# montyhall/bot7

Measured on AMD Instinct MI355X. Metric: EI candidates scored/sec at N=2048,d=32, higher is better.
Workload: dtype f64

## Files before the change

### bot7_amd/csrc/b7_internal.h

```cpp
#pragma once
#include <hip/hip_runtime.h>
#include <stddef.h>
#include <stdint.h>

#include <map>
#include <string>
#include <vector>

#include "bot7hip.h"

constexpr int B7_NPAD = 128;
constexpr int B7_PANEL = 64;
constexpr int B7_PERSIST_NMAX = 4096;
constexpr int B7_MROWS = 256;
constexpr int B7_MAX_D = 96;

constexpr int B7_TAB_VAL = 0;
constexpr int B7_TAB_IDX = 1;
constexpr int B7_TAB_STATUS = 2;
constexpr int B7_TAB_ROWS = 3;
constexpr int B7_TAB_ROW0 = 4;
constexpr int B7_TAB_W = B7_TAB_ROW0 + B7_MAX_D;
constexpr int B7_MAX_WORLD = 64;

static inline int b7_dpad_class(int d) {
  return d <= 4 ? 4 : d <= 8 ? 8 : d <= 16 ? 16 : d <= 32 ? 32 : d <= 48 ? 48 : d <= 64 ? 64 : 96;
}

constexpr size_t B7_INFO_HEAD_BYTES = 16 + sizeof(double) * 257 + 8;
constexpr size_t B7_PERSIST_FLAG_WORDS_MAX = 16 + 2 * 64 * 64 + 2 * 64;
constexpr size_t B7_INFO_BYTES = B7_INFO_HEAD_BYTES + 4 * B7_PERSIST_FLAG_WORDS_MAX;

struct DevBuf {
  void *p = nullptr;
  size_t cap = 0;
};

struct PinBuf {
  void *host = nullptr, *dev = nullptr;
  size_t bytes = 0;
};

struct FitBlock { int info[4]; double terms[257]; };
struct BestPair { double v; int64_t i; };
constexpr int SOBOL_DIMS = 40;
constexpr int SOBOL_BITS = 30;
struct SobolTable {
  uint32_t v[SOBOL_DIMS][SOBOL_BITS];
};

constexpr size_t B7_PINNED_BYTES = 16384;
struct PinnedBlock {
  FitBlock fit;
  alignas(256) BestPair best;
  alignas(4096) double fmin[256];
  alignas(4096) double vec[B7_MAX_D + 3];
};
static_assert(offsetof(PinnedBlock, fit) == 0 && offsetof(PinnedBlock, best) == 2304 && offsetof(PinnedBlock, fmin) == 4096 &&
                  offsetof(PinnedBlock, vec) == 8192 && sizeof(PinnedBlock) <= B7_PINNED_BYTES,
              "pinned block: kernels and copies address these slots");

constexpr size_t B7_SCRATCH_BYTES = 64 * 1024;
struct ScratchBlock {
  double lenscale[256];
  double fmin[256];
  SobolTable sobol;
  double minmax[2 * B7_MAX_D];
  alignas(4096) double colvec[2 * B7_MAX_D];
};
static_assert(offsetof(ScratchBlock, lenscale) == 0 && offsetof(ScratchBlock, fmin) == 2048 && offsetof(ScratchBlock, sobol) == 4096 &&
                  offsetof(ScratchBlock, minmax) == 4096 + sizeof(SobolTable) && offsetof(ScratchBlock, colvec) == 12288 &&
                  sizeof(ScratchBlock) <= B7_SCRATCH_BYTES,
              "scratch block: the layout every earlier build used");

constexpr int B7_ACC_NONE = 0, B7_ACC_LINEAR = 1, B7_ACC_LOG = 2;

struct PhaseStat {
  double ms = 0.0;
  int64_t launches = 0;
};

struct ScoreParams {
  int kind = 0, S = 0, upper = 0, nlev = 0;
  const double *mu = nullptr, *var = nullptr;
  union {
    const double *fmin = nullptr;
    const double *ystar;
  };
  long long stride = 0;
  double fmin0 = 0.0, tradeoff = 0.0, sign = 0.0;
};

struct b7_ctx {
  int device = 0;
  hipStream_t stream = nullptr;
  hipEvent_t ev_fit = nullptr;
  std::string err;
  int cus = 0;

  DevBuf grid[2];
  int grid_cur = 0;
  int64_t M = 0;
  int d = 0;

  bool fitted = false;
  bool have_data = false;
  int model_kind = 0;
  int N = 0, Npad = 0, dfit = 0, dpad = 0, ycols = 0;
  int yld = 1;
  double amp = 0, noise = 0, mean = 0;
  b7_gp_opts opts;
  int kernel = B7_KERNEL_ARDSE;
  DevBuf xobs;
  DevBuf w;
  DevBuf zsc;
  DevBuf zss;
  DevBuf K;
  DevBuf L;
  DevBuf Linv;
  DevBuf W;
  DevBuf dinv;
  DevBuf alpha;
  DevBuf resid;
  DevBuf atmp;
  DevBuf info;
  DevBuf ybuf;

  bool predicted = false;
  int64_t Mpred = 0;
  DevBuf mu;
  DevBuf var;
  DevBuf acc;
  bool acc_valid = false;
  int spin_us = 500;
  bool npad_small = true;
  bool potrf_small = true;
  bool blr_small = true;
  double fmin_scalar = 0.0;
  bool acc_fresh = false;
  int acc_kind = 0;
  DevBuf ks;
  size_t ks_bytes = (size_t)4 << 30;
  int diag_variant = 1;
  int inverse_inline = 1;
  PinnedBlock *pinned = nullptr, *pinned_dev = nullptr;
  std::vector<double> net_host;
  PinBuf pin_blr;
  PinBuf pin_eval;
  PinBuf pin_nll;
  bool fmin_staged = false;
  bool potrf_attrs_set = false;
  bool linv_done = false;
  int potrf_sched = 3;
  int syrk_small = 1;
  int potrf_defer = 1;
  int potrf_group = 2;
  struct JobList { DevBuf buf; int n = 0; };
  std::map<int, JobList> pjobs_cache;
  DevBuf pstamps;
  int pjobs_nb = 0, pjobs_n = 0;
  DevBuf bhyp, bw, bzsc, bzss, bK, bL, bdinv, bflags, binfo, bresid, bterms, bLinv, balpha, bmu, bvar;
  bool persist_attr_set = false, persist_stamps = false;
  int persist_helpers = 0;
  int persist_aborts = 0;
  int nll_small = 1;
  bool kpost_small = true;
  bool fit_small = true;
  int persist_fault = -1;
  int potrf_sched_saved = 0;
  DevBuf part;
  DevBuf ystar, mes_ticket;
  DevBuf mes_user;
  int mes_levels = 8;
  int mes_S = 0, mes_K = 0, mes_nb = 0;
  int64_t mes_M = 0;
  int mes_slot = 0;
  bool mes_valid = false;
  DevBuf ticket;
  DevBuf scratch;
  DevBuf tmpgrid;
  DevBuf tmpmu, tmpvar;
  DevBuf fant;
  DevBuf bel;
  DevBuf belvec;
  PinBuf pin_bel;
  DevBuf feat;
  size_t feat_zeroed_bytes = 0;
  int feat_z = -1;
  int64_t Mfeat = 0;
  int zdim = 0;
  uint64_t feat_version = 0, grid_version = 0;
  DevBuf netbuf;

  void *comm = nullptr;
  int comm_rank = 0, comm_world = 1;
  DevBuf slots;
  uint64_t *tab_host = nullptr;
  uint64_t *tab_host_dev = nullptr;
  struct b7_group *group = nullptr;
  bool group_busy = false;
  bool win_valid = false;
  int64_t win_idx1 = 0;
  int win_rank = -1, win_d = 0;
  double win_row[B7_MAX_D];
  int64_t shard_rows[B7_MAX_WORLD];
  int shard_world = 0;

  hipEvent_t tev[B7_MAX_TIMERS][2];
  bool tev_init = false;
  bool profile = false;
  std::map<std::string, PhaseStat> phases;
  struct PendingPhase { const char *name; hipEvent_t e0, e1; };
  std::vector<PendingPhase> pending;
  std::vector<hipEvent_t> free_events;
  hipEvent_t phase_e0 = nullptr;
};

int b7_fail(b7_ctx *c, int code, const char *fmt, ...);
#define B7_HIP(c, expr)                                                                          \
  do {                                                                                           \
    hipError_t e__ = (expr);                                                                     \
    if (e__ != hipSuccess)                                                                       \
      return b7_fail((c), e__ == hipErrorOutOfMemory ? B7_ERR_NOMEM : B7_ERR_HIP, "%s:%d: %s", \
                     __FILE_NAME__, __LINE__, hipGetErrorString(e__));                           \
  } while (0)
#define B7_TRY(expr)          \
  do {                        \
    int rc__ = (expr);        \
    if (rc__ != B7_OK) return rc__; \
  } while (0)

int b7_ensure(b7_ctx *c, DevBuf &b, size_t bytes);
void b7_release(DevBuf &b);
int b7_pin_ensure(b7_ctx *c, PinBuf &b, size_t bytes, bool mapped);
static inline ScratchBlock *b7_scratch(const b7_ctx *c) { return static_cast<ScratchBlock *>(c->scratch.p); }

struct PhaseScope {
  b7_ctx *c;
  const char *name;
  PhaseScope(b7_ctx *c, const char *name);
  ~PhaseScope();
};

static inline int64_t round_up(int64_t x, int64_t m) { return (x + m - 1) / m * m; }
int npad_of(const b7_ctx *c, int64_t n);

int launch_sobol(b7_ctx *c, double *out, int64_t size, int dims, int64_t skip, const double *mins,
                 const double *maxes);
int launch_random_grid(b7_ctx *c, double *out, int64_t size, int dims, uint64_t seed, int64_t row_offset,
                       const double *mins, const double *maxes);
int launch_remove_row(b7_ctx *c, const double *src, double *dst, int64_t M, int d, int64_t idx0);
int launch_remove_rows(b7_ctx *c, const double *src, double *dst, int64_t M, int d, const int64_t *cuts_dev, int ncut);
int launch_colrange(b7_ctx *c, const double *grid, int64_t M, int d, double *out_dev);
int launch_col_affine(b7_ctx *c, double *grid, int64_t M, int d, const double *v_dev, bool mul);
int launch_gather_rows(b7_ctx *c, const double *src, double *out, const int64_t *idx0_dev, int64_t n, int d);

struct KBatchDesc {
  int64_t s_w = 0, s_zsc = 0, s_zsh = 0, s_out = 0;
  const double *amp = nullptr;
  int64_t s_alpha = 0, s_mu = 0;
  const double *mean = nullptr;
};
struct ObsSet {
  const double *zsc;
  const double *zsh;
  int npad;
  const double *w = nullptr;
  KBatchDesc batch;
};
int launch_prep_obs_aux(b7_ctx *c, const double *xobs, const double *ls_dev, int N, int npad, double *zsc,
                        double *zsh);
int launch_k_generic(b7_ctx *c, const double *xq, int64_t rows, int64_t Mtotal, const ObsSet &o, double *out);
int launch_prep_obs(b7_ctx *c, const double *xobs, const double *lenscale_sq_dev, int N, int d);
int launch_kxx(b7_ctx *c, double diag_add);
int launch_ksx_batch(b7_ctx *c, int S, const double *xq, int64_t rows, int64_t Mtotal, const double *w, const double *zsc,
                     const double *zss, const double *amp_dev, const double *mean_dev, const double *alpha, double *ks,
                     int64_t s_out, double *mu, int64_t s_mu);
int launch_kxx_batch(b7_ctx *c, int B, const double *ls_dev, const double *amp_dev, const double *noise_dev, double *w,
                     double *zsc, double *zss, double *K);
int launch_ksx(b7_ctx *c, const double *xq, int64_t row0, int64_t rows, int64_t Mtotal, int d, double *ks,
               double *mu, int ycols);

struct FactorNote {
  bool alpha_done = false;
  int *report_written = nullptr;
};
int launch_potrf(b7_ctx *c, double extra, bool with_inverse, int *report_hint = nullptr, FactorNote *note = nullptr);
int launch_trtri(b7_ctx *c);
int launch_potrf_persist(b7_ctx *c, double extra, bool with_inverse);
int launch_nll_batch(b7_ctx *c, int B, const double *K, double *L, double *dinv, unsigned *flags, int *info,
                     const double *resid, double *terms);
int launch_nll_one(b7_ctx *c, const double *K, double *L, double *dinv, unsigned *flags, int *info, const double *resid,
                   double *terms, double extra);
size_t persist_flag_words_host(int nb);
int launch_potrf_small(b7_ctx *c, int B, const double *K, double *L, double *Linv, double *dinv, const double *resid, double *alpha,
                       double extra, int *info, int *report_dev, int64_t sK, int64_t sL, int64_t sdinv, int64_t svec, int sinfo);
int launch_blr_head_small(b7_ctx *c, const double *Z, int N, int z, int ldz, const double *yv, double alpha_prec, double beta,
                          int *report_dev);
int launch_blr_heads_small(b7_ctx *c, int S, const double *Z, int N, int z, int ldz, const double *yraw_dev, const double *hyp3_dev,
                           double *L, double *Linv, double *m, double *b, int *info, int *report_dev, double *terms);
int launch_post_heads(b7_ctx *c, int S, const double *Linv, const double *feat, int64_t rows, int64_t Mtotal, double *var, int64_t svar,
                      const double *zero_dev, const double *invbeta_dev);
int launch_gemv_rows_batch(b7_ctx *c, int S, const double *A, int lda, const double *x, int64_t sx, int n, const double *base_dev,
                           int64_t rows, double *y, int64_t sy);
int launch_nll_small(b7_ctx *c, int B, const double *hyp_dev, const double *hyp_host, double *terms_dev, int *info_dev,
                     unsigned *done_dev);
bool kpost_small_applies(const b7_ctx *c);
int launch_kpost_small(b7_ctx *c, int S, const double *xq, int64_t M, const double *w, const double *zsc, const double *zss,
                       const double *Linv, const double *alpha, const double *hyp_dev, double amp, double noise, double mean,
                       double *mu, double *var, int64_t sout);
bool gp_small_applies(const b7_ctx *c);
static inline bool fit_small_applies(const b7_ctx *c) {
  return c->fit_small && c->potrf_sched == 3 && c->inverse_inline && gp_small_applies(c);
}
int launch_nll_small8(b7_ctx *c, int B, const double *hyp_dev, const double *hyp_host, double *terms_dev, int *info_dev,
                      unsigned *done_dev);
int launch_fit_small(b7_ctx *c, int B, const double *hyp_dev, const double *hyp_host, double *hyp_out, double *w, double *zsc,
                     double *zss, double *L, double *Linv, double *dinv, double *alpha, double *resid, int *info_dev,
                     int *report_dev);
int launch_alpha(b7_ctx *c, int *report_dev = nullptr, int report_words = 0, const FactorNote &note = FactorNote());
int launch_alpha_batch(b7_ctx *c, int B, const double *Linv, const double *resid, double *alpha, const int *report_src = nullptr,
                       int *report_dev = nullptr, int report_words = 0);
int launch_fit_batch(b7_ctx *c, int B, const double *K, double *L, double *Linv, double *dinv, unsigned *flags, int *info);
int launch_nll_terms(b7_ctx *c, double *out_dev);
int launch_fro_norm_sq(b7_ctx *c, const double *A, int n, int ld, double *out_dev);
int launch_set_identity(b7_ctx *c);

int launch_post(b7_ctx *c, const double *ks, int64_t row0, int64_t rows, int64_t Mtotal, double *var);
int launch_post_batch(b7_ctx *c, int S, const double *Linv, const double *ks, int64_t sks, int64_t rows, int64_t Mtotal,
                      double *var, int64_t svar, const double *amp_dev, const double *noise_dev);

int launch_mean_multi(b7_ctx *c, const double *ks, int64_t row0, int64_t rows, int64_t Mtotal, double *mu);
int launch_gemm_nt(b7_ctx *c, const double *A, int lda, const double *B, int ldb, double *C, int ldc, int m, int n,
                   int k);
int launch_fantasy_cov(b7_ctx *c, const double *kpp, const double *g, double *S, int P, double diag_add);
int launch_fantasy_factor(b7_ctx *c, double *S, double *dinv_tmp, int *info_dev);
int launch_fantasy_sample(b7_ctx *c, const double *Lp, const double *mu, int P, int n, uint64_t seed, double *out);
int launch_add_diag(b7_ctx *c, double *S, int ld, int n, double v);

int launch_append_finalize(b7_ctx *c, const double *krow, const double *lvec, const double *uvec, const double *evec,
                           int *status_dev);
int launch_append_vectors(b7_ctx *c, const double *krow, double *lvec, double *uvec, double *part, double *evec);
int launch_mlp_forward(b7_ctx *c, const double *X, int64_t M, int d, const double *net_dev, const int *dims,
                       int n_layers, int activation, double *out, int ld_out);
int launch_mlp_forward_mean(b7_ctx *c, const double *X, int64_t M, int d, const double *net_dev, const int *dims,
                            int n_layers, int activation, double *out, int ld_out, const double *mvec, double mean0,
                            double *mu, bool *mean_done);
int launch_gemv_rows(b7_ctx *c, const double *A, int lda, const double *x, int n, double base, int64_t row0,
                     int64_t rows, int64_t Mtotal, double *y);
int launch_transpose_pad(b7_ctx *c, const double *Z, int n, int ldz, int z, double *Zt, int zpad, int nk);
int launch_blr_assemble(b7_ctx *c, const double *G, double *K, int z, int zpad, double alpha_prec, double beta);

int launch_score(b7_ctx *c, ScoreParams p, const double *mu, const double *var, int64_t M, int ycols, double *out, bool accumulate);
int launch_score_batch(b7_ctx *c, const ScoreParams &p, double *acc, int64_t M);
int launch_finish(b7_ctx *c, double *acc, int64_t M, double divisor, double *best_val, int64_t *best_idx1, bool logacc = false);
int launch_fill(b7_ctx *c, double *p, int64_t n, double v);
int launch_finish_slot(b7_ctx *c, double *acc, int64_t M, double divisor, uint64_t *tab_dev, int rank, int world,
                       int64_t offset, const double *grid, int d, bool all_slots, uint64_t *host_rec = nullptr,
                       unsigned *host_done = nullptr, bool logacc = false);

struct ExclRows {
  int n = 0;
  long long row[B7_BATCH_MAX];
};
int launch_score_finish_slot(b7_ctx *c, const ScoreParams &p, double *acc, int64_t M, double divisor, uint64_t *tab_dev,
                             int rank, int world, int64_t offset, const double *grid, int d, bool all_slots, uint64_t *host_rec = nullptr,
                             unsigned *host_done = nullptr, const ExclRows *excl = nullptr);
void acc_declare_zeros(b7_ctx *c, int score_kind);
int acc_write_zeros(b7_ctx *c);
void acc_forget(b7_ctx *c);
int acc_materialize(b7_ctx *c);
int launch_keep_record(b7_ctx *c, uint64_t *tab_dev, int rank, int world);
int launch_row_slot(b7_ctx *c, uint64_t *tab_dev, int rank, int world, int64_t idx1_global, int64_t local0, const double *grid,
                    int d);

int exch_table_ensure(b7_ctx *c, int world);
int exch_local(b7_ctx *c, double divisor, int64_t offset, int rank, int world, bool all_slots, bool mirror = false,
               const ScoreParams *pend = nullptr, const ExclRows *excl = nullptr);
int exch_wait_mirror(b7_ctx *c);
int exch_fail_record(b7_ctx *c, int rank, int world, int code);
int exch_allreduce(b7_ctx *c);
int exch_collective(b7_ctx *c, int rc, int rank, int world, double *best_val, int64_t *best_idx1);
int exch_rewrite_record(b7_ctx *c, int rank, int world);
int exch_fetch(b7_ctx *c, int first_rank, int nranks);
bool exch_pick(const uint64_t *tab, int world, int stride, double *val, int64_t *idx1, int *rank);
int exch_conclude(b7_ctx *c, const uint64_t *tab, int world, double *best_val, int64_t *best_idx1);
void exch_forget(b7_ctx *c);

void persist_gave_up(b7_ctx *c);
int chol_with_jitter(b7_ctx *c, double *jitter_out, int *info_first_out, bool with_inverse, FactorNote *note = nullptr);
int check_hyp(b7_ctx *c, const b7_hyp *hyp, int d);
void launch_resid_batch(b7_ctx *c, int B, const double *mean_dev);
int fit_front(b7_ctx *c, const b7_hyp *hyp, const double *ls_dev);
int fit_hyp_core(b7_ctx *c, const b7_hyp *hyp, double *nll_out, double *jitter_used, int *info_out, bool then_predict);
int64_t predict_chunk(const b7_ctx *c, int64_t M);
int predict_into(b7_ctx *c, const double *xq, int64_t M, double *mu, double *var);
int copy_out_mu_var(b7_ctx *c, const void *mu, const void *var, int64_t M, int cols, double *mean_host, double *var_host,
                    bool wait = false);

struct HypPack { double *ls, *amp, *noise, *mean; };
static inline HypPack hyp_pack(void *base, int B, int d) {
  double *amp = static_cast<double *>(base) + (size_t)B * d;
  return {static_cast<double *>(base), amp, amp + B, amp + 2 * (size_t)B};
}

int nominate_args(b7_ctx *c, const char *who, const b7_score_spec *spec, int64_t offset);
int stage_fmin(b7_ctx *c, const double *fmin, double **fd_out);
static inline bool score_needs_fmin(int kind) { return kind == B7_SCORE_EI || kind == B7_SCORE_LOGEI; }
constexpr int score_acc_kind(int kind) { return kind == B7_SCORE_LOGEI ? B7_ACC_LOG : B7_ACC_LINEAR; }
int mes_begin(b7_ctx *c, int S, int64_t M, int K);
int launch_mes_search(b7_ctx *c, const double *mu, const double *var, int64_t stride, int nS, int slot0);
const double *mes_ystar_dev(const b7_ctx *c, int slot);
int mes_refuse(b7_ctx *c, const char *who, const b7_score_spec *spec);
ScoreParams score_params(const b7_ctx *c, const b7_score_spec *spec, const double *fd);
int score_add(b7_ctx *c, const b7_score_spec *sp, const double *fd, bool accumulate = true);
int pending_score(b7_ctx *c, int S, const b7_score_spec *spec, const double *fd, ScoreParams *out);
int eval_validate(b7_ctx *c, int S, const b7_hyp *hyps, const b7_score_spec *spec, int64_t offset);
struct BelKeep {
  double *mu = nullptr, *var = nullptr;
  const double *w = nullptr, *zsc = nullptr, *zss = nullptr, *Linv = nullptr;
};
int eval_enqueue(b7_ctx *c, int S, const b7_hyp *hyps, const b7_score_spec *spec, ScoreParams *pend, BelKeep *keep = nullptr);
bool reports_clean(b7_ctx *c, const int *reports, int S, bool persist);
int eval_redo(b7_ctx *c, int S, const b7_hyp *hyps, const b7_score_spec *spec, double *jitter_out, int *info_out,
              BelKeep *keep = nullptr);
struct BelPass {
  const double *xq; int64_t rows;
  const double *xj;
  const double *w, *zsc, *zss;
  const double *wj;
  const double *par;
  double *scal;
  double *kcol;
  double *var, *u; int64_t sgrid;
  int64_t idx; int j;
};
int launch_believer(b7_ctx *c, int S, const BelPass &p, bool column);
int grid_drop_row(b7_ctx *c, int64_t local_idx1, double *row_out_sync);

template <class Enqueue, class Clean, class Redo>
static inline int nominate_run(b7_ctx *c, const char *who, int rc, int64_t offset, double divisor, Enqueue enqueue, Clean clean,
                        Redo redo, double *best_val, int64_t *best_idx1) {
  const int world = c->comm ? c->comm_world : 1, rank = c->comm ? c->comm_rank : 0;
  ScoreParams pend;
  if (!(c->comm && c->comm_world > 1)) {
    B7_TRY(rc);
    B7_TRY(enqueue(&pend));
    B7_TRY(exch_local(c, divisor, offset, rank, world, true, true, &pend));
    B7_TRY(exch_wait_mirror(c));
    if (!clean()) {
      B7_TRY(redo());
      B7_TRY(exch_local(c, divisor, offset, rank, world, true, true));
      B7_TRY(exch_wait_mirror(c));
    }
    return exch_conclude(c, c->tab_host, world, best_val, best_idx1);
  }
  if (rc == B7_OK && c->M > 0) {
    rc = enqueue(&pend);
    if (rc == B7_OK) rc = hipStreamSynchronize(c->stream) == hipSuccess ? B7_OK : b7_fail(c, B7_ERR_HIP, "%s: stream failed", who);
    if (rc == B7_OK && !clean()) {
      pend = ScoreParams();
      rc = redo();
    }
  }
  if (rc == B7_OK) rc = exch_local(c, divisor, offset, rank, world, true, false, &pend);
  return exch_collective(c, rc, rank, world, best_val, best_idx1);
}
```

### bot7_amd/csrc/context.hip

```cpp
#include <stdarg.h>
#include <stdio.h>
#include <stdlib.h>
#include <string.h>

#include "b7_internal.h"

static thread_local std::string g_create_err;

int b7_fail(b7_ctx *c, int code, const char *fmt, ...) {
  char buf[512];
  va_list ap;
  va_start(ap, fmt);
  vsnprintf(buf, sizeof(buf), fmt, ap);
  va_end(ap);
  if (c)
    c->err = buf;
  else
    g_create_err = buf;
  return code;
}

int b7_ensure(b7_ctx *c, DevBuf &b, size_t bytes) {
  if (bytes == 0) bytes = 16;
  if (b.cap >= bytes) return B7_OK;
  if (b.p) {
    B7_HIP(c, hipStreamSynchronize(c->stream));
    B7_HIP(c, hipFree(b.p));
    b.p = nullptr;
    b.cap = 0;
  }
  hipError_t e = hipMalloc(&b.p, bytes);
  if (e != hipSuccess) {
    b.p = nullptr;
    return b7_fail(c, B7_ERR_NOMEM, "hipMalloc(%zu bytes): %s", bytes, hipGetErrorString(e));
  }
  b.cap = bytes;
  return B7_OK;
}

void b7_release(DevBuf &b) {
  if (b.p) (void)hipFree(b.p);
  b.p = nullptr;
  b.cap = 0;
}

int b7_pin_ensure(b7_ctx *c, PinBuf &b, size_t bytes, bool mapped) {
  if (b.bytes >= bytes) return B7_OK;
  B7_HIP(c, hipStreamSynchronize(c->stream));
  if (b.host) (void)hipHostFree(b.host);
  b = PinBuf();
  B7_HIP(c, hipHostMalloc(&b.host, 2 * bytes, mapped ? hipHostMallocMapped : hipHostMallocDefault));
  if (mapped) B7_HIP(c, hipHostGetDevicePointer(&b.dev, b.host, 0));
  b.bytes = 2 * bytes;
  return B7_OK;
}

static hipEvent_t phase_event(b7_ctx *c) {
  if (!c->free_events.empty()) {
    hipEvent_t e = c->free_events.back();
    c->free_events.pop_back();
    return e;
  }
  hipEvent_t e = nullptr;
  (void)hipEventCreate(&e);
  return e;
}

static void resolve_phases(b7_ctx *c) {
  if (c->pending.empty()) return;
  (void)hipStreamSynchronize(c->stream);
  for (const b7_ctx::PendingPhase &p : c->pending) {
    float ms = 0.f;
    if (p.e0 && p.e1 && hipEventElapsedTime(&ms, p.e0, p.e1) == hipSuccess) {
      PhaseStat &s = c->phases[p.name];
      s.ms += ms;
      s.launches += 1;
    }
    if (p.e0) c->free_events.push_back(p.e0);
    if (p.e1) c->free_events.push_back(p.e1);
  }
  c->pending.clear();
}

PhaseScope::PhaseScope(b7_ctx *c_, const char *name_) : c(c_), name(name_) {
  if (!c->profile) return;
  c->phase_e0 = phase_event(c);
  if (c->phase_e0) (void)hipEventRecord(c->phase_e0, c->stream);
}
PhaseScope::~PhaseScope() {
  if (!c->profile || !c->phase_e0) return;
  hipEvent_t e1 = phase_event(c);
  if (e1) (void)hipEventRecord(e1, c->stream);
  c->pending.push_back({name, c->phase_e0, e1});
  c->phase_e0 = nullptr;
  if (c->pending.size() >= 4096) resolve_phases(c);
}

int npad_of(const b7_ctx *c, int64_t n) { return (c->npad_small && n <= 64) ? 64 : (int)round_up(n, B7_NPAD); }

static int timers_init(b7_ctx *c) {
  if (c->tev_init) return B7_OK;
  for (int i = 0; i < B7_MAX_TIMERS; ++i) {
    B7_HIP(c, hipEventCreate(&c->tev[i][0]));
    B7_HIP(c, hipEventCreate(&c->tev[i][1]));
  }
  c->tev_init = true;
  return B7_OK;
}

extern "C" {

int b7_abi_version(void) { return B7_ABI_VERSION; }

int b7_create(b7_ctx **out, int device_id) {
  if (!out) return b7_fail(nullptr, B7_ERR_INVALID, "b7_create: out is NULL");
  *out = nullptr;
  int ndev = 0;
  hipError_t e = hipGetDeviceCount(&ndev);
  if (e != hipSuccess || ndev <= 0)
    return b7_fail(nullptr, B7_ERR_HIP, "no HIP device available (%s); libbot7hip has no CPU path",
                   e == hipSuccess ? "device count 0" : hipGetErrorString(e));
  if (device_id < 0 || device_id >= ndev)
    return b7_fail(nullptr, B7_ERR_INVALID, "device_id %d out of range [0,%d)", device_id, ndev);
  e = hipSetDevice(device_id);
  if (e != hipSuccess) return b7_fail(nullptr, B7_ERR_HIP, "hipSetDevice: %s", hipGetErrorString(e));
  hipDeviceProp_t prop;
  e = hipGetDeviceProperties(&prop, device_id);
  if (e != hipSuccess) return b7_fail(nullptr, B7_ERR_HIP, "hipGetDeviceProperties: %s", hipGetErrorString(e));
  if (strncmp(prop.gcnArchName, "gfx950", 6) != 0)
    return b7_fail(nullptr, B7_ERR_UNSUPPORTED, "device %d is %s; libbot7hip is built for gfx950 only", device_id,
                   prop.gcnArchName);
  b7_ctx *c = new b7_ctx();
  c->device = device_id;
  c->cus = prop.multiProcessorCount;
  b7_gp_default_opts(&c->opts);
  if (const char *pv = getenv("B7_SPIN_US")) c->spin_us = atoi(pv);
#ifdef B7_DIAG
  if (const char *pv = getenv("B7_DIAG_VARIANT")) c->diag_variant = atoi(pv);
  if (const char *pv = getenv("B7_NPAD_SMALL")) c->npad_small = atoi(pv) != 0;
  if (const char *pv = getenv("B7_POTRF_SMALL")) c->potrf_small = atoi(pv) != 0;
  if (getenv("B7_POTRF_SCHED") || getenv("B7_DIAG_VARIANT") || getenv("B7_INVERSE_INLINE")) c->potrf_small = c->fit_small = false;
  if (const char *pv = getenv("B7_BLR_SMALL")) c->blr_small = atoi(pv) != 0;
  if (const char *pv = getenv("B7_INVERSE_INLINE")) c->inverse_inline = atoi(pv);
  if (const char *pv = getenv("B7_POTRF_SCHED")) c->potrf_sched = atoi(pv);
  c->persist_stamps = getenv("B7_PERSIST_STAMPS") != nullptr;
  if (const char *pv = getenv("B7_PERSIST_HELPERS")) c->persist_helpers = atoi(pv);
  if (const char *pv = getenv("B7_PERSIST_FAULT")) c->persist_fault = atoi(pv);
  if (const char *pv = getenv("B7_NLL_SMALL")) c->nll_small = atoi(pv);
  if (const char *pv = getenv("B7_FIT_SMALL")) c->fit_small = atoi(pv) != 0;
  if (const char *pv = getenv("B7_KPOST_SMALL")) c->kpost_small = atoi(pv) != 0;
  if (const char *pv = getenv("B7_SYRK_SMALL")) c->syrk_small = atoi(pv) ? 1 : 0;
  if (const char *pv = getenv("B7_POTRF_DEFER")) c->potrf_defer = atoi(pv) ? 1 : 0;
  if (const char *pv = getenv("B7_POTRF_GROUP")) {
    const int g = atoi(pv);
    if (g >= 1 && g <= 8) c->potrf_group = g;
  }
#endif
  e = hipStreamCreateWithFlags(&c->stream, hipStreamNonBlocking);
  if (e == hipSuccess) e = hipEventCreateWithFlags(&c->ev_fit, hipEventDisableTiming);
  if (e == hipSuccess) e = hipHostMalloc((void **)&c->pinned, B7_PINNED_BYTES, hipHostMallocMapped);
  if (e == hipSuccess) e = hipHostGetDevicePointer((void **)&c->pinned_dev, c->pinned, 0);
  if (e != hipSuccess) {
    if (c->pinned) (void)hipHostFree(c->pinned);
    if (c->stream) (void)hipStreamDestroy(c->stream);
    delete c;
    return b7_fail(nullptr, B7_ERR_HIP, "stream / pinned result block creation: %s", hipGetErrorString(e));
  }
  if (b7_ensure(c, c->scratch, B7_SCRATCH_BYTES) != B7_OK) {
    g_create_err = c->err;
    b7_destroy(c);
    return B7_ERR_NOMEM;
  }
  *out = c;
  return B7_OK;
}

void b7_destroy(b7_ctx *c) {
  if (!c) return;
  (void)hipSetDevice(c->device);
  (void)hipStreamSynchronize(c->stream);
  (void)b7_comm_destroy(c);
  DevBuf *all[] = {&c->grid[0], &c->grid[1], &c->xobs, &c->w,     &c->zsc,  &c->zss,     &c->K,      &c->L,
                   &c->Linv,    &c->W,       &c->dinv, &c->alpha, &c->resid, &c->info,   &c->ybuf,   &c->mu,
                   &c->var,     &c->acc,     &c->ks,   &c->part,  &c->scratch, &c->tmpgrid, &c->tmpmu, &c->tmpvar, &c->fant, &c->feat, &c->netbuf, &c->atmp, &c->slots, &c->pstamps,
                   &c->bhyp, &c->bw, &c->bzsc, &c->bzss, &c->bK, &c->bL, &c->bdinv, &c->bflags, &c->binfo, &c->bresid, &c->bterms,
                   &c->bLinv, &c->balpha, &c->bmu, &c->bvar, &c->ticket, &c->bel, &c->belvec, &c->ystar, &c->mes_ticket, &c->mes_user};
  for (auto &kv : c->pjobs_cache) b7_release(kv.second.buf);
  for (DevBuf *b : all) b7_release(*b);
  if (c->tev_init)
    for (int i = 0; i < B7_MAX_TIMERS; ++i) {
      (void)hipEventDestroy(c->tev[i][0]);
      (void)hipEventDestroy(c->tev[i][1]);
    }
  resolve_phases(c);
  if (c->pinned) (void)hipHostFree(c->pinned);
  for (PinBuf *b : {&c->pin_eval, &c->pin_blr, &c->pin_nll, &c->pin_bel})
    if (b->host) (void)hipHostFree(b->host);
  if (c->tab_host) (void)hipHostFree(c->tab_host);
  for (hipEvent_t e : c->free_events) (void)hipEventDestroy(e);
  if (c->phase_e0) (void)hipEventDestroy(c->phase_e0);
  if (c->ev_fit) (void)hipEventDestroy(c->ev_fit);
  (void)hipStreamDestroy(c->stream);
  delete c;
}

const char *b7_last_error(const b7_ctx *c) { return c ? c->err.c_str() : g_create_err.c_str(); }

int b7_device_info(b7_ctx *c, char *name_out, int *compute_units, int64_t *hbm_bytes) {
  if (!c) return B7_ERR_INVALID;
  hipDeviceProp_t prop;
  B7_HIP(c, hipGetDeviceProperties(&prop, c->device));
  if (name_out) snprintf(name_out, 64, "%s (%s)", prop.name, prop.gcnArchName);
  if (compute_units) *compute_units = prop.multiProcessorCount;
  if (hbm_bytes) *hbm_bytes = (int64_t)prop.totalGlobalMem;
  return B7_OK;
}

int b7_sync(b7_ctx *c) {
  if (!c) return B7_ERR_INVALID;
  B7_HIP(c, hipStreamSynchronize(c->stream));
  return B7_OK;
}

int b7_set_workspace(b7_ctx *c, int64_t bytes) {
  if (!c || bytes < (int64_t)(8 * 128 * 128)) return c ? b7_fail(c, B7_ERR_INVALID, "workspace too small") : B7_ERR_INVALID;
  c->ks_bytes = (size_t)bytes;
  return B7_OK;
}

int b7_timer_start(b7_ctx *c, int slot) {
  if (!c || slot < 0 || slot >= B7_MAX_TIMERS) return B7_ERR_INVALID;
  B7_TRY(timers_init(c));
  B7_HIP(c, hipEventRecord(c->tev[slot][0], c->stream));
  return B7_OK;
}

int b7_timer_stop(b7_ctx *c, int slot) {
  if (!c || slot < 0 || slot >= B7_MAX_TIMERS) return B7_ERR_INVALID;
  B7_TRY(timers_init(c));
  B7_HIP(c, hipEventRecord(c->tev[slot][1], c->stream));
  return B7_OK;
}

int b7_timer_ms(b7_ctx *c, int slot, float *ms_out) {
  if (!c || slot < 0 || slot >= B7_MAX_TIMERS || !ms_out) return B7_ERR_INVALID;
  B7_TRY(timers_init(c));
  B7_HIP(c, hipEventSynchronize(c->tev[slot][1]));
  B7_HIP(c, hipEventElapsedTime(ms_out, c->tev[slot][0], c->tev[slot][1]));
  return B7_OK;
}

int b7_profile_enable(b7_ctx *c, int on) {
  if (!c) return B7_ERR_INVALID;
  c->profile = on != 0;
  return B7_OK;
}

int b7_profile_reset(b7_ctx *c) {
  if (!c) return B7_ERR_INVALID;
  resolve_phases(c);
  c->phases.clear();
  return B7_OK;
}

int b7_profile_get(b7_ctx *c, const char *phase, double *ms_total, int64_t *launches) {
  if (!c || !phase) return B7_ERR_INVALID;
  resolve_phases(c);
  auto it = c->phases.find(phase);
  if (ms_total) *ms_total = it == c->phases.end() ? 0.0 : it->second.ms;
  if (launches) *launches = it == c->phases.end() ? 0 : it->second.launches;
  return B7_OK;
}

}
```

### bot7_amd/csrc/covar.hip

```cpp
#include "b7_internal.h"
#include "gemm_f64.h"
#include "ksx_exp.h"

namespace {

__constant__ double exp2_tab_dev[128];

__global__ void __launch_bounds__(64) prep_obs_kernel(const double *__restrict__ xobs, const double *ls, double *w,
                                                      double *zsc, double *zsh, int N, int Npad, int d, int dpad) {
  extern __shared__ __align__(16) double psm[];
  {
    const int64_t b = blockIdx.y;
    ls += b * d;
    w += b * dpad;
    zsc += b * (int64_t)Npad * dpad;
    zsh += b * Npad;
  }
  const int tld = dpad + 1, lane = threadIdx.x, row0 = blockIdx.x * 64;
  double *tile = psm, *wl = psm + 64 * tld;
  for (int k = lane; k < dpad; k += 64) {
    const double wk = (k < d) ? 1.0 / ls[k] : 0.0;
    wl[k] = wk;
    if (blockIdx.x == 0) w[k] = wk;
  }
  int nrows = N - row0;
  nrows = nrows < 0 ? 0 : (nrows > 64 ? 64 : nrows);
  const double *src = xobs + (int64_t)row0 * d;
#pragma unroll 8
  for (int e = lane; e < nrows * d; e += 64) {
    const int r = e / d, k = e - r * d;
    tile[r * tld + k] = src[e];
  }
  __syncthreads();
  double s = 0.0;
#pragma unroll 8
  for (int k = 0; k < dpad; ++k) {
    const double z = (lane < nrows && k < d) ? tile[lane * tld + k] : 0.0;
    const double wk = wl[k];
    tile[lane * tld + k] = z * wk;
    s += (z * z) * wk;
  }
  if (row0 + lane < Npad) zsh[row0 + lane] = (lane < nrows) ? 0.5 * s : 1e300;
  __syncthreads();
  double *dst = zsc + (int64_t)row0 * dpad;
#pragma unroll 8
  for (int e = lane; e < 64 * dpad; e += 64) {
    const int r = e / dpad, k = e - r * dpad;
    if (row0 + r < Npad) dst[e] = tile[r * tld + k];
  }
}

__device__ __forceinline__ void pair_pack(double a, double b, d2_t &out) {
  const int alo = __double2loint(a), ahi = __double2hiint(a), blo = __double2loint(b), bhi = __double2hiint(b);
  int o0l, o0h, o1l, o1h;
  asm volatile(
      "s_mov_b32 vcc_lo, 0x55555555\n\t"
      "s_mov_b32 vcc_hi, 0x55555555\n\t"
      "s_nop 0\n\t"
      "v_cndmask_b32_dpp %0, %6, %4, vcc quad_perm:[1,0,3,2] row_mask:0xf bank_mask:0xf\n\t"
      "v_cndmask_b32_dpp %1, %7, %5, vcc quad_perm:[1,0,3,2] row_mask:0xf bank_mask:0xf\n\t"
      "s_not_b64 vcc, vcc\n\t"
      "v_cndmask_b32_dpp %2, %4, %6, vcc quad_perm:[1,0,3,2] row_mask:0xf bank_mask:0xf\n\t"
      "v_cndmask_b32_dpp %3, %5, %7, vcc quad_perm:[1,0,3,2] row_mask:0xf bank_mask:0xf"
      : "=&v"(o0l), "=&v"(o0h), "=&v"(o1l), "=&v"(o1h)
      : "v"(alo), "v"(ahi), "v"(blo), "v"(bhi)
      : "vcc", "scc");
  out[0] = __hiloint2double(o0h, o0l);
  out[1] = __hiloint2double(o1h, o1l);
}

constexpr int KQ = 64;
__host__ __device__ constexpr int ksx_slab(int dpad) { return dpad >= 48 ? 32 : 64; }

using KBatch = KBatchDesc;
template <int DPAD, int KERN>
__global__ void __launch_bounds__(256)
    ksx_kernel(const double *__restrict__ xq, int64_t row0, int64_t Mtotal, int d, int dpad_rt, const double *w,
               const double *zsc, const double *zsh, const double *__restrict__ alpha, double amp, double meanc, int Npad,
               double *out, double *__restrict__ mu, KBatch kb) {
  extern __shared__ __align__(16) double sm[];
  if (kb.amp) {
    const int64_t bz = blockIdx.z;
    w += bz * kb.s_w;
    zsc += bz * kb.s_zsc;
    zsh += bz * kb.s_zsh;
    out += bz * kb.s_out;
    amp = kb.amp[bz];
    if (kb.mean) {
      alpha += bz * kb.s_alpha;
      mu += bz * kb.s_mu;
      meanc = kb.mean[bz];
    }
  }
  constexpr int KO = ksx_slab(DPAD);
  constexpr int TPR = 256 / KO;
  constexpr int dpad = DPAD, NCH = (DPAD / 2 + TPR - 1) / TPR, KSTEPS = DPAD / 4;
  constexpr int stride = DPAD + 1;
  (void)dpad_rt;
  constexpr int R0 = (KQ * stride > 2 * KO * stride) ? KQ * stride : 2 * KO * stride;
  double *sq = sm;
  double *so = sm;
  double *sh = sm + R0;
  double *sal = sh + 2 * KO;
  double *shq = sal + 2 * KO;
  double *stab = shq + KQ;
  const int tid = threadIdx.x, lane = tid & 63, wave = tid >> 6;
  const int lr = lane & 15, lq = lane >> 4;
  const int64_t qbase = row0 + (int64_t)blockIdx.x * KQ;
  const int srow = tid / TPR, sq4 = tid % TPR;
  const int qrow = tid >> 2, qq4 = tid & 3;
  constexpr int half = DPAD >> 1;

  if (tid < 128) stab[tid] = amp * exp2_tab_dev[tid];
  {
    int64_t g = qbase + qrow;
    if (g > Mtotal - 1) g = Mtotal - 1;
    for (int k = qq4; k < dpad; k += 4) sq[qrow * stride + k] = (k < d) ? xq[g * d + k] : 0.0;
  }
  const int nslab_total = Npad / KO;
  const int nslab = nslab_total / gridDim.y;
  const int slab0 = blockIdx.y * nslab;

  d2_t pre[NCH];
  double pre_h = 0.0, pre_a = 0.0;
  auto load_slab = [&](int s) {
    const double *src = zsc + (int64_t)(s * KO + srow) * dpad;
#pragma unroll
    for (int i = 0; i < NCH; ++i) {
      const int kc = i * TPR + sq4;
      if (kc < half) pre[i] = *reinterpret_cast<const d2_t *>(src + 2 * kc);
    }
    if (tid < KO) {
      pre_h = zsh[s * KO + tid];
      pre_a = alpha ? alpha[s * KO + tid] : 0.0;
    }
  };
  auto store_slab = [&](int buf) {
    double *dst = so + buf * KO * stride + srow * stride;
#pragma unroll
    for (int i = 0; i < NCH; ++i) {
      const int kc = i * TPR + sq4;
      if (kc < half) {
        dst[2 * kc] = pre[i][0];
        dst[2 * kc + 1] = pre[i][1];
      }
    }
    if (tid < KO) {
      sh[buf * KO + tid] = pre_h;
      sal[buf * KO + tid] = pre_a;
    }
  };

  load_slab(slab0);
  __syncthreads();
  if (tid < KQ) {
    double s = 0.0;
    for (int k = 0; k < dpad; ++k) {
      double x = sq[tid * stride + k];
      s += (x * x) * w[k];
    }
    shq[tid] = 0.5 * s;
  }
  double qf[KSTEPS];
#pragma unroll
  for (int k4 = 0; k4 < KSTEPS; ++k4) qf[k4] = sq[(wave * 16 + lr) * stride + lq + 4 * k4];
  __syncthreads();
  store_slab(0);
  __syncthreads();

  double hq[4], macc[4] = {0.0, 0.0, 0.0, 0.0};
#pragma unroll
  for (int r = 0; r < 4; ++r) hq[r] = shq[wave * 16 + lq + 4 * r];
  const bool odd = lane & 1;
  double *orow = out + ((int64_t)blockIdx.x * KQ + wave * 16 + lq + (odd ? 4 : 0)) * Npad + (lr & ~1);

  int cur = 0;
  for (int s = 0; s < nslab; ++s) {
    const bool more = (s + 1) < nslab;
    if (more) load_slab(slab0 + s + 1);
    const double *sob = so + cur * KO * stride;
    const int o0 = (slab0 + s) * KO;
#pragma unroll
    for (int t = 0; t < KO / 16; ++t) {
      const double *ob = sob + (t * 16 + lr) * stride + lq;
      d4_t c = {0.0, 0.0, 0.0, 0.0};
      {
        double bf[KSTEPS];
#pragma unroll
        for (int k4 = 0; k4 < KSTEPS; ++k4) bf[k4] = ob[4 * k4];
#if B7_KSX_ABLATE & 8
        c = mfma_f64(qf[0], bf[0], c);
#else
#pragma unroll
        for (int k4 = 0; k4 < KSTEPS; ++k4) c = mfma_f64(qf[k4], bf[k4], c);
#endif
      }
      const double hk = sh[cur * KO + t * 16 + lr];
      const double al = sal[cur * KO + t * 16 + lr];
      double kv[4], arg[4];
#pragma unroll
      for (int r = 0; r < 4; ++r) arg[r] = (c[r] - hq[r]) - hk;
#if B7_KSX_ABLATE & 4
#pragma unroll
      for (int r = 0; r < 4; ++r) kv[r] = arg[r];
#else
      cov_nonpos4<KERN>(arg, stab, kv);
#endif
#pragma unroll
      for (int r = 0; r < 4; ++r) macc[r] = __builtin_fma(kv[r], al, macc[r]);
      d2_t v01, v23;
      pair_pack(kv[0], kv[1], v01);
      pair_pack(kv[2], kv[3], v23);
      {
        double *p = orow + o0 + t * 16;
#if B7_KSX_ABLATE & 1
        if (v01[0] == 1.2345e-300) {
#endif
#if B7_KSX_ABLATE & 16
        double *pi = out + ((int64_t)blockIdx.x * KQ + wave * 16 + 4 * t + (lane >> 5)) * Npad + o0 + (lane & 31) * 2;
        *reinterpret_cast<d2_t *>(pi) = v01;
        *reinterpret_cast<d2_t *>(pi + (int64_t)2 * Npad) = v23;
#elif B7_KSX_ABLATE & 32
        __builtin_nontemporal_store(v01, reinterpret_cast<d2_t *>(p));
        __builtin_nontemporal_store(v23, reinterpret_cast<d2_t *>(p + (int64_t)8 * Npad));
#else
        *reinterpret_cast<d2_t *>(p) = v01;
        *reinterpret_cast<d2_t *>(p + (int64_t)8 * Npad) = v23;
#endif
#if B7_KSX_ABLATE & 1
        }
#endif
      }
    }
    if (more) store_slab(cur ^ 1);
    __syncthreads();
    cur ^= 1;
  }

  if (mu) {
#pragma unroll
    for (int r = 0; r < 4; ++r) {
      double v = macc[r];
      v += __shfl_xor(v, 1);
      v += __shfl_xor(v, 2);
      v += __shfl_xor(v, 4);
      v += __shfl_xor(v, 8);
      const int64_t g = qbase + wave * 16 + lq + 4 * r;
      if (lr == 0 && g < Mtotal) mu[g] = meanc + v;
    }
  }
}

__global__ void __launch_bounds__(256)
    kxx_fix_kernel(double *K, int N, int Npad, double diag_add, const double *diag_arr, int64_t sK) {
  if (diag_arr) {
    K += (int64_t)blockIdx.y * sK;
    diag_add = diag_arr[blockIdx.y];
  }
  int64_t e = (int64_t)blockIdx.x * blockDim.x + threadIdx.x;
  if (e >= (int64_t)Npad * Npad) return;
  int i = (int)(e / Npad), j = (int)(e - (int64_t)i * Npad);
  if (i >= N || j >= N)
    K[e] = (i == j) ? 1.0 : 0.0;
  else if (i == j)
    K[e] += diag_add;
}

size_t ksx_lds_bytes(int dpad) {
  const int KO = ksx_slab(dpad);
  const size_t r0 = (size_t)(KQ > 2 * KO ? KQ : 2 * KO) * (dpad + 1);
  size_t bytes = sizeof(double) * (r0 + 4 * KO + KQ + 128);
#if B7_KSX_ABLATE & 128
  const size_t per_cu = 160 * 1024, fit = per_cu / bytes;
  if (fit > 1) bytes = per_cu / (fit - 1) - 512;
#endif
  return bytes;
}

int ensure_exp_table(b7_ctx *c) {
  static bool done[64] = {false};
  if (c->device < 64 && done[c->device]) return B7_OK;
  B7_HIP(c, hipMemcpyToSymbol(HIP_SYMBOL(exp2_tab_dev), b7_exp2_tab, sizeof(b7_exp2_tab)));
  if (c->device < 64) done[c->device] = true;
  return B7_OK;
}

template <int DPAD, int KERN>
int ksx_launch(b7_ctx *c, dim3 grid, const double *xq, int64_t row0, int64_t Mtotal, int d, const ObsSet &o,
               const double *alpha, double meanc, double *out, double *mu) {
  const size_t lds = ksx_lds_bytes(DPAD);
  auto kern = ksx_kernel<DPAD, KERN>;
  B7_TRY(ensure_exp_table(c));
  B7_HIP(c, hipFuncSetAttribute(reinterpret_cast<const void *>(kern), hipFuncAttributeMaxDynamicSharedMemorySize,
                                (int)lds));
  hipLaunchKernelGGL(kern, grid, dim3(256), lds, c->stream, xq, row0, Mtotal, d, c->dpad, o.w ? o.w : (const double *)c->w.p,
                     o.zsc, o.zsh, alpha, c->amp, meanc, o.npad, out, mu, o.batch);
  B7_HIP(c, hipGetLastError());
  return B7_OK;
}

template <int KERN>
int ksx_dispatch_k(b7_ctx *c, dim3 grid, const double *xq, int64_t row0, int64_t Mtotal, int d, const ObsSet &o,
                   const double *alpha, double meanc, double *out, double *mu) {
  switch (c->dpad) {
    case 4: return ksx_launch<4, KERN>(c, grid, xq, row0, Mtotal, d, o, alpha, meanc, out, mu);
    case 8: return ksx_launch<8, KERN>(c, grid, xq, row0, Mtotal, d, o, alpha, meanc, out, mu);
    case 16: return ksx_launch<16, KERN>(c, grid, xq, row0, Mtotal, d, o, alpha, meanc, out, mu);
    case 32: return ksx_launch<32, KERN>(c, grid, xq, row0, Mtotal, d, o, alpha, meanc, out, mu);
    case 48: return ksx_launch<48, KERN>(c, grid, xq, row0, Mtotal, d, o, alpha, meanc, out, mu);
    case 64: return ksx_launch<64, KERN>(c, grid, xq, row0, Mtotal, d, o, alpha, meanc, out, mu);
    case 96: return ksx_launch<96, KERN>(c, grid, xq, row0, Mtotal, d, o, alpha, meanc, out, mu);
    default: return b7_fail(c, B7_ERR_UNSUPPORTED, "covariance kernel: dpad %d is not a built class", c->dpad);
  }
}

int ksx_dispatch(b7_ctx *c, dim3 grid, const double *xq, int64_t row0, int64_t Mtotal, int d, const ObsSet &o,
                 const double *alpha, double meanc, double *out, double *mu) {
  if (c->kernel == B7_KERNEL_MATERN52) return ksx_dispatch_k<B7_KERNEL_MATERN52>(c, grid, xq, row0, Mtotal, d, o, alpha, meanc, out, mu);
  return ksx_dispatch_k<B7_KERNEL_ARDSE>(c, grid, xq, row0, Mtotal, d, o, alpha, meanc, out, mu);
}

}

int launch_prep_obs(b7_ctx *c, const double *xobs, const double *ls_dev, int N, int d) {
  PhaseScope ps(c, "prep");
  const size_t lds = sizeof(double) * (64 * (size_t)(c->dpad + 1) + c->dpad);
  hipLaunchKernelGGL(prep_obs_kernel, dim3((c->Npad + 63) / 64), dim3(64), lds, c->stream, xobs, ls_dev,
                     (double *)c->w.p, (double *)c->zsc.p, (double *)c->zss.p, N, c->Npad, d, c->dpad);
  B7_HIP(c, hipGetLastError());
  return B7_OK;
}

int launch_prep_obs_aux(b7_ctx *c, const double *xobs, const double *ls_dev, int N, int npad, double *zsc,
                        double *zsh) {
  const size_t lds = sizeof(double) * (64 * (size_t)(c->dpad + 1) + c->dpad);
  hipLaunchKernelGGL(prep_obs_kernel, dim3((npad + 63) / 64), dim3(64), lds, c->stream, xobs, ls_dev, (double *)c->w.p,
                     zsc, zsh, N, npad, c->dfit, c->dpad);
  B7_HIP(c, hipGetLastError());
  return B7_OK;
}

int launch_k_generic(b7_ctx *c, const double *xq, int64_t rows, int64_t Mtotal, const ObsSet &o, double *out) {
  if (rows % KQ || o.npad % 64) return b7_fail(c, B7_ERR_INVALID, "k_generic: extents not multiples of 64");
  return ksx_dispatch(c, dim3((unsigned)(rows / KQ), 1), xq, 0, Mtotal, c->dfit, o, nullptr, 0.0, out, nullptr);
}

int launch_ksx(b7_ctx *c, const double *xq, int64_t row0, int64_t rows, int64_t Mtotal, int d, double *ks,
               double *mu, int ycols) {
  PhaseScope ps(c, "ksx");
  if (rows % KQ) return b7_fail(c, B7_ERR_INVALID, "ksx: rows %lld not a multiple of %d", (long long)rows, KQ);
  if (ycols != 1) mu = nullptr;
  const ObsSet o{(const double *)c->zsc.p, (const double *)c->zss.p, c->Npad};
  return ksx_dispatch(c, dim3((unsigned)(rows / KQ), 1), xq, row0, Mtotal, d, o,
                      mu ? (const double *)c->alpha.p : nullptr, c->mean, ks, mu);
}

int launch_kxx(b7_ctx *c, double diag_add) {
  PhaseScope ps(c, "kxx");
  const int Npad = c->Npad;
  int ny = 1;
  while (ny < 16 && (Npad / 64) % (ny * 2) == 0 && (Npad / KQ) * ny < 2 * c->cus) ny *= 2;
  const ObsSet o{(const double *)c->zsc.p, (const double *)c->zss.p, Npad};
  B7_TRY(ksx_dispatch(c, dim3(Npad / KQ, ny), (const double *)c->xobs.p, 0, c->N, c->dfit, o, nullptr, 0.0,
                      (double *)c->K.p, nullptr));
  int64_t total = (int64_t)Npad * Npad;
  hipLaunchKernelGGL(kxx_fix_kernel, dim3((unsigned)((total + 255) / 256)), dim3(256), 0, c->stream, (double *)c->K.p,
                     c->N, Npad, diag_add, (const double *)nullptr, (int64_t)0);
  B7_HIP(c, hipGetLastError());
  return B7_OK;
}

int launch_ksx_batch(b7_ctx *c, int S, const double *xq, int64_t rows, int64_t Mtotal, const double *w, const double *zsc,
                     const double *zss, const double *amp_dev, const double *mean_dev, const double *alpha, double *ks,
                     int64_t s_out, double *mu, int64_t s_mu) {
  PhaseScope ps(c, "ksx");
  if (rows % KQ) return b7_fail(c, B7_ERR_INVALID, "ksx: rows %lld not a multiple of %d", (long long)rows, KQ);
  ObsSet o{zsc, zss, c->Npad};
  o.w = w;
  o.batch.s_w = c->dpad;
  o.batch.s_zsc = (int64_t)c->Npad * c->dpad;
  o.batch.s_zsh = c->Npad;
  o.batch.s_out = s_out;
  o.batch.amp = amp_dev;
  o.batch.s_alpha = c->Npad;
  o.batch.s_mu = s_mu;
  o.batch.mean = mean_dev;
  return ksx_dispatch(c, dim3((unsigned)(rows / KQ), 1, S), xq, 0, Mtotal, c->dfit, o, alpha, 0.0, ks, mu);
}

int launch_kxx_batch(b7_ctx *c, int B, const double *ls_dev, const double *amp_dev, const double *noise_dev, double *w,
                     double *zsc, double *zss, double *K) {
  PhaseScope ps(c, "kxx");
  const int Npad = c->Npad, d = c->dfit, dpad = c->dpad;
  const size_t lds = sizeof(double) * (64 * (size_t)(dpad + 1) + dpad);
  hipLaunchKernelGGL(prep_obs_kernel, dim3((Npad + 63) / 64, B), dim3(64), lds, c->stream, (const double *)c->xobs.p, ls_dev,
                     w, zsc, zss, c->N, Npad, d, dpad);
  ObsSet o{zsc, zss, Npad};
  o.w = w;
  o.batch.s_w = dpad;
  o.batch.s_zsc = (int64_t)Npad * dpad;
  o.batch.s_zsh = Npad;
  o.batch.s_out = (int64_t)Npad * Npad;
  o.batch.amp = amp_dev;
  int ny = 1;
  while (ny < 16 && (Npad / 64) % (ny * 2) == 0 && (Npad / KQ) * ny * B < 2 * c->cus) ny *= 2;
  B7_TRY(ksx_dispatch(c, dim3(Npad / KQ, ny, B), (const double *)c->xobs.p, 0, c->N, d, o, nullptr, 0.0, K, nullptr));
  const int64_t total = (int64_t)Npad * Npad;
  hipLaunchKernelGGL(kxx_fix_kernel, dim3((unsigned)((total + 255) / 256), B), dim3(256), 0, c->stream, K, c->N, Npad, 0.0,
                     noise_dev, total);
  B7_HIP(c, hipGetLastError());
  return B7_OK;
}
```

Before: 16.06 million.

## Software-pipeline LDS fragment loads ahead of MFMAs in covariance kernel

```diff
diff --git a/bot7_amd/csrc/b7_internal.h b/bot7_amd/csrc/b7_internal.h
--- a/bot7_amd/csrc/b7_internal.h
+++ b/bot7_amd/csrc/b7_internal.h
@@ -165,6 +165,7 @@
   int persist_aborts = 0;
   int nll_small = 1;
   bool kpost_small = true;
+  int ksx_loop = -1;
   bool fit_small = true;
   int persist_fault = -1;
   int potrf_sched_saved = 0;
diff --git a/bot7_amd/csrc/context.hip b/bot7_amd/csrc/context.hip
--- a/bot7_amd/csrc/context.hip
+++ b/bot7_amd/csrc/context.hip
@@ -149,6 +149,7 @@
   if (const char *pv = getenv("B7_NLL_SMALL")) c->nll_small = atoi(pv);
   if (const char *pv = getenv("B7_FIT_SMALL")) c->fit_small = atoi(pv) != 0;
   if (const char *pv = getenv("B7_KPOST_SMALL")) c->kpost_small = atoi(pv) != 0;
+  if (const char *pv = getenv("B7_KSX_LOOP")) c->ksx_loop = atoi(pv) != 0;
   if (const char *pv = getenv("B7_SYRK_SMALL")) c->syrk_small = atoi(pv) ? 1 : 0;
   if (const char *pv = getenv("B7_POTRF_DEFER")) c->potrf_defer = atoi(pv) ? 1 : 0;
   if (const char *pv = getenv("B7_POTRF_GROUP")) {
diff --git a/bot7_amd/csrc/covar.hip b/bot7_amd/csrc/covar.hip
--- a/bot7_amd/csrc/covar.hip
+++ b/bot7_amd/csrc/covar.hip
@@ -73,7 +73,9 @@
 __host__ __device__ constexpr int ksx_slab(int dpad) { return dpad >= 48 ? 32 : 64; }
 
 using KBatch = KBatchDesc;
-template <int DPAD, int KERN>
+__host__ __device__ constexpr int ksx_ahead(int dpad) { return dpad >= 96 ? 4 : dpad / 4 < 8 ? dpad / 4 : 8; }
+
+template <int DPAD, int KERN, bool PIPE>
 __global__ void __launch_bounds__(256)
     ksx_kernel(const double *__restrict__ xq, int64_t row0, int64_t Mtotal, int d, int dpad_rt, const double *w,
                const double *zsc, const double *zsh, const double *__restrict__ alpha, double amp, double meanc, int Npad,
@@ -174,67 +176,121 @@
   const bool odd = lane & 1;
   double *orow = out + ((int64_t)blockIdx.x * KQ + wave * 16 + lq + (odd ? 4 : 0)) * Npad + (lr & ~1);
 
+  auto epilogue = [&](const d4_t &c, double hk, double al, double *p) {
+    double kv[4], arg[4];
+#pragma unroll
+    for (int r = 0; r < 4; ++r) arg[r] = (c[r] - hq[r]) - hk;
+#if B7_KSX_ABLATE & 4
+#pragma unroll
+    for (int r = 0; r < 4; ++r) kv[r] = arg[r];
+#else
+    cov_nonpos4<KERN>(arg, stab, kv);
+#endif
+#pragma unroll
+    for (int r = 0; r < 4; ++r) macc[r] = __builtin_fma(kv[r], al, macc[r]);
+    d2_t v01, v23;
+    pair_pack(kv[0], kv[1], v01);
+    pair_pack(kv[2], kv[3], v23);
+#if B7_KSX_ABLATE & 1
+    if (v01[0] == 1.2345e-300) {
+#endif
+#if B7_KSX_ABLATE & 16
+    const int64_t col = p - orow;
+    double *pi = out + ((int64_t)blockIdx.x * KQ + wave * 16 + (col & (KO - 1)) / 4 + (lane >> 5)) * Npad + (col & ~(int64_t)(KO - 1)) + (lane & 31) * 2;
+    *reinterpret_cast<d2_t *>(pi) = v01;
+    *reinterpret_cast<d2_t *>(pi + (int64_t)2 * Npad) = v23;
+#elif B7_KSX_ABLATE & 32
+    __builtin_nontemporal_store(v01, reinterpret_cast<d2_t *>(p));
+    __builtin_nontemporal_store(v23, reinterpret_cast<d2_t *>(p + (int64_t)8 * Npad));
+#else
+    *reinterpret_cast<d2_t *>(p) = v01;
+    *reinterpret_cast<d2_t *>(p + (int64_t)8 * Npad) = v23;
+#endif
+#if B7_KSX_ABLATE & 1
+    }
+#endif
+  };
+
+  constexpr int T = KO / 16;
   int cur = 0;
-  for (int s = 0; s < nslab; ++s) {
-    const bool more = (s + 1) < nslab;
-    if (more) load_slab(slab0 + s + 1);
-    const double *sob = so + cur * KO * stride;
-    const int o0 = (slab0 + s) * KO;
-#pragma unroll
-    for (int t = 0; t < KO / 16; ++t) {
-      const double *ob = sob + (t * 16 + lr) * stride + lq;
-      d4_t c = {0.0, 0.0, 0.0, 0.0};
-      {
-        double bf[KSTEPS];
-#pragma unroll
-        for (int k4 = 0; k4 < KSTEPS; ++k4) bf[k4] = ob[4 * k4];
+  if constexpr (!PIPE) {
+    for (int s = 0; s < nslab; ++s) {
+      const bool more = (s + 1) < nslab;
+      if (more) load_slab(slab0 + s + 1);
+      const double *sob = so + cur * KO * stride;
+      const int o0 = (slab0 + s) * KO;
+#pragma unroll
+      for (int t = 0; t < T; ++t) {
+        const double *ob = sob + (t * 16 + lr) * stride + lq;
+        d4_t c = {0.0, 0.0, 0.0, 0.0};
+        {
+          double bf[KSTEPS];
+#pragma unroll
+          for (int k4 = 0; k4 < KSTEPS; ++k4) bf[k4] = ob[4 * k4];
 #if B7_KSX_ABLATE & 8
-        c = mfma_f64(qf[0], bf[0], c);
+          c = mfma_f64(qf[0], bf[0], c);
 #else
 #pragma unroll
-        for (int k4 = 0; k4 < KSTEPS; ++k4) c = mfma_f64(qf[k4], bf[k4], c);
-#endif
+          for (int k4 = 0; k4 < KSTEPS; ++k4) c = mfma_f64(qf[k4], bf[k4], c);
+#endif
+        }
+        const double hk = sh[cur * KO + t * 16 + lr];
+        const double al = sal[cur * KO + t * 16 + lr];
+        epilogue(c, hk, al, orow + o0 + t * 16);
       }
-      const double hk = sh[cur * KO + t * 16 + lr];
-      const double al = sal[cur * KO + t * 16 + lr];
-      double kv[4], arg[4];
-#pragma unroll
-      for (int r = 0; r < 4; ++r) arg[r] = (c[r] - hq[r]) - hk;
-#if B7_KSX_ABLATE & 4
-#pragma unroll
-      for (int r = 0; r < 4; ++r) kv[r] = arg[r];
-#else
-      cov_nonpos4<KERN>(arg, stab, kv);
-#endif
-#pragma unroll
-      for (int r = 0; r < 4; ++r) macc[r] = __builtin_fma(kv[r], al, macc[r]);
-      d2_t v01, v23;
-      pair_pack(kv[0], kv[1], v01);
-      pair_pack(kv[2], kv[3], v23);
-      {
-        double *p = orow + o0 + t * 16;
-#if B7_KSX_ABLATE & 1
-        if (v01[0] == 1.2345e-300) {
-#endif
-#if B7_KSX_ABLATE & 16
-        double *pi = out + ((int64_t)blockIdx.x * KQ + wave * 16 + 4 * t + (lane >> 5)) * Npad + o0 + (lane & 31) * 2;
-        *reinterpret_cast<d2_t *>(pi) = v01;
-        *reinterpret_cast<d2_t *>(pi + (int64_t)2 * Npad) = v23;
-#elif B7_KSX_ABLATE & 32
-        __builtin_nontemporal_store(v01, reinterpret_cast<d2_t *>(p));
-        __builtin_nontemporal_store(v23, reinterpret_cast<d2_t *>(p + (int64_t)8 * Npad));
-#else
-        *reinterpret_cast<d2_t *>(p) = v01;
-        *reinterpret_cast<d2_t *>(p + (int64_t)8 * Npad) = v23;
-#endif
-#if B7_KSX_ABLATE & 1
+      if (more) store_slab(cur ^ 1);
+      __syncthreads();
+      cur ^= 1;
+    }
+  } else {
+    constexpr int AHEAD = ksx_ahead(DPAD), GRP = AHEAD >= 2 ? 2 : 1;
+    static_assert(KSTEPS % GRP == 0 && AHEAD % GRP == 0 && (T * KSTEPS) % AHEAD == 0, "fragment ring");
+    double bf[AHEAD];
+    auto first_frags = [&](const double *sob) {
+      const double *ob = sob + lr * stride + lq;
+#pragma unroll
+      for (int i = 0; i < AHEAD; ++i) bf[i] = ob[4 * i];
+    };
+    first_frags(so);
+    B7_STAGE();
+    for (int s = 0; s < nslab; ++s) {
+      const bool more = (s + 1) < nslab;
+      if (more) load_slab(slab0 + s + 1);
+      const double *sob = so + cur * KO * stride;
+      const int o0 = (slab0 + s) * KO;
+      d4_t c;
+      double hk, al;
+#pragma unroll
+      for (int t = 0; t < T; ++t) {
+        const double *ob = sob + (t * 16 + lr) * stride + lq;
+        hk = sh[cur * KO + t * 16 + lr];
+        al = sal[cur * KO + t * 16 + lr];
+        B7_STAGE();
+        c = d4_t{0.0, 0.0, 0.0, 0.0};
+#pragma unroll
+        for (int k4 = 0; k4 < KSTEPS; ++k4) {
+          if (!(B7_KSX_ABLATE & 8) || k4 == 0) c = mfma_f64(qf[k4], bf[(t * KSTEPS + k4) % AHEAD], c);
+          if (k4 % GRP == GRP - 1) {
+#pragma unroll
+            for (int j = k4 - GRP + 1; j <= k4; ++j) {
+              const int f = j + AHEAD;
+              if (f < KSTEPS)
+                bf[(t * KSTEPS + j) % AHEAD] = ob[4 * f];
+              else if (t + 1 < T)
+                bf[(t * KSTEPS + j) % AHEAD] = ob[16 * stride + 4 * (f - KSTEPS)];
+            }
+            B7_STAGE();
+          }
         }
-#endif
+        if (t + 1 < T) epilogue(c, hk, al, orow + o0 + t * 16);
       }
-    }
-    if (more) store_slab(cur ^ 1);
-    __syncthreads();
-    cur ^= 1;
+      if (more) store_slab(cur ^ 1);
+      __syncthreads();
+      cur ^= 1;
+      if (more) first_frags(so + cur * KO * stride);
+      B7_STAGE();
+      epilogue(c, hk, al, orow + o0 + (T - 1) * 16);
+    }
   }
 
   if (mu) {
@@ -285,11 +341,13 @@
   return B7_OK;
 }
 
-template <int DPAD, int KERN>
-int ksx_launch(b7_ctx *c, dim3 grid, const double *xq, int64_t row0, int64_t Mtotal, int d, const ObsSet &o,
-               const double *alpha, double meanc, double *out, double *mu) {
+constexpr bool ksx_pipelined(int dpad) { return dpad == 32 || dpad == 96; }
+
+template <int DPAD, int KERN, bool PIPE>
+int ksx_launch_as(b7_ctx *c, dim3 grid, const double *xq, int64_t row0, int64_t Mtotal, int d, const ObsSet &o,
+                  const double *alpha, double meanc, double *out, double *mu) {
   const size_t lds = ksx_lds_bytes(DPAD);
-  auto kern = ksx_kernel<DPAD, KERN>;
+  auto kern = ksx_kernel<DPAD, KERN, PIPE>;
   B7_TRY(ensure_exp_table(c));
   B7_HIP(c, hipFuncSetAttribute(reinterpret_cast<const void *>(kern), hipFuncAttributeMaxDynamicSharedMemorySize,
                                 (int)lds));
@@ -297,6 +355,16 @@
                      o.zsc, o.zsh, alpha, c->amp, meanc, o.npad, out, mu, o.batch);
   B7_HIP(c, hipGetLastError());
   return B7_OK;
+}
+
+template <int DPAD, int KERN>
+int ksx_launch(b7_ctx *c, dim3 grid, const double *xq, int64_t row0, int64_t Mtotal, int d, const ObsSet &o,
+               const double *alpha, double meanc, double *out, double *mu) {
+#ifdef B7_DIAG
+  if (c->ksx_loop >= 0 && (c->ksx_loop != 0) != ksx_pipelined(DPAD))
+    return ksx_launch_as<DPAD, KERN, !ksx_pipelined(DPAD)>(c, grid, xq, row0, Mtotal, d, o, alpha, meanc, out, mu);
+#endif
+  return ksx_launch_as<DPAD, KERN, ksx_pipelined(DPAD)>(c, grid, xq, row0, Mtotal, d, o, alpha, meanc, out, mu);
 }
 
 template <int KERN>
```

Result: no change. 16.03 million (-0.2%).
